# Pi-Star-Lab/RESCO

Hardware: AMD Instinct MI355X
Metric: env-steps/sec (higher is better)
Workload: dtype f32; 1 GPU; ingolstadt21 x 4096 lock-step envs per GPU (BASELINE config 3), fixed demand from the map's rou.xml, on-device seeded random policy, Krauss sigma 0.5 + speedFactor dev 0.1; tls_expiry=1, map=ingolstadt21, envs_per_gpu=4096, pipes=2, ticks_per_env_step=10, block_threads=512, lds_bytes_per_env=40896, parallelism=env-batch split x1, no collective on the data path

## Files before the change

resco_amd/csrc/resco_step.h:

```cpp
#pragma once
#include "resco_tables.h"

struct State {
    char *base;
    size_t nc;
    int32_t *trip_log;
    int32_t *env;
    int32_t *tls;
    long long *stats;
    uint16_t *dep_next;
    uint32_t *mail;
    RS_HD float *pos() const { return (float *)base; }
    RS_HD float *speed() const { return RS_G((float *)(base + 4 * nc)); }
    RS_HD float *accel() const { return RS_G((float *)(base + 8 * nc)); }
    RS_HD float *tloss() const { return RS_G((float *)(base + 12 * nc)); }
    RS_HD float *sf() const { return RS_G((float *)(base + 16 * nc)); }
    RS_HD uint32_t *coop(int par) const { return RS_G((uint32_t *)(base + (par ? 43 : 20) * nc)); }
    RS_HD uint32_t *cooplead(int par) const { return RS_G((uint32_t *)(base + (par ? 47 : 24) * nc)); }
    RS_HD uint16_t *lane() const { return RS_G((uint16_t *)(base + 28 * nc)); }
    RS_HD uint16_t *trip() const { return RS_G((uint16_t *)(base + 30 * nc)); }
    RS_HD uint16_t *cursor() const { return RS_G((uint16_t *)(base + 32 * nc)); }
    RS_HD uint16_t *swait() const { return RS_G((uint16_t *)(base + 34 * nc)); }
    RS_HD uint16_t *rwait() const { return RS_G((uint16_t *)(base + 36 * nc)); }
    RS_HD uint16_t *depart() const { return RS_G((uint16_t *)(base + 38 * nc)); }
// ... 345 lines not shown
    const int waves = C >= 768 ? 8 : ((C / 2) + 63) / 64;
    return (waves * 64 == 512 && lds <= RS_LDS_4WG_LIMIT) ? V64 : V80;
}
RS_CARVE void scn_consts_layout(ScnConsts *c, const Lds &L, size_t lds_bytes) {
#define X(n, tp) c->o_##n = L.n.off;
    RS_SCN_LDS(X)
#undef X
    c->gstride = L.gstride; c->lcap = L.lcap; c->lds_bytes = (uint32_t)lds_bytes;
    __builtin_memcpy(&c->cell_inv_bits, &L.cell_inv, 4);
}
template <class F> RS_CARVE bool scn_fix_matches(const ScnConsts &c) {
    bool ok = c.cell_inv_bits == F::cell_inv_bits && c.gstride == F::gstride && c.lcap == F::lcap && c.lds_bytes == F::lds_bytes && c.budget == F::budget;
#define X(n) ok = ok && c.n == F::n;
    RS_SCN_KTAB(X)
#undef X
#define X(n) ok = ok && c.n##_bits == F::n##_bits;
    RS_SCN_KTAB_F(X)
#undef X
#define X(n, tp) ok = ok && c.o_##n == F::o_##n;
    RS_SCN_LDS(X)
#undef X
    return ok;
}

struct StepArgs { KTab T; State G; Out O; Lds L; StateP GP; };

template <int DEM, class TT> struct Demand {
    const TT &T;
    const uint32_t off;
    RS_MEM Demand(const TT &T_, int env) : T(T_), off(DEM == 1 || (DEM == 2 && T_.dem()) ? rs_at(T_.dem_env(), env) : 0u) {}
    template <class Tp> RS_MEM const Tp *at(uint32_t o) const { return (const Tp *)(T.dem() + (off + o)); }
    RS_MEM const int32_t *trip_depart() const { if constexpr (DEM == 1) return at<int32_t>(dem_off_depart(T.n_trips, T.n_dep, T.horizon)); else if constexpr (DEM == 2) return T.dem() ? at<int32_t>(dem_off_depart(T.n_trips, T.n_dep, T.horizon)) : T.cold.trip_depart; else return T.cold.trip_depart; }
    RS_MEM const int32_t *trips_cum() const { if constexpr (DEM == 1) return at<int32_t>(dem_off_cum(T.n_trips, T.n_dep, T.horizon)); else if constexpr (DEM == 2) return T.dem() ? at<int32_t>(dem_off_cum(T.n_trips, T.n_dep, T.horizon)) : T.cold.trips_cum; else return T.cold.trips_cum; }
    RS_MEM const uint16_t *trip_next() const { if constexpr (DEM == 1) return at<uint16_t>(dem_off_next(T.n_trips, T.n_dep, T.horizon)); else if constexpr (DEM == 2) return T.dem() ? at<uint16_t>(dem_off_next(T.n_trips, T.n_dep, T.horizon)) : T.cold.trip_next; else return T.cold.trip_next; }
    RS_MEM const uint16_t *trip_route() const { if constexpr (DEM == 1) return at<uint16_t>(dem_off_route(T.n_trips, T.n_dep, T.horizon)); else if constexpr (DEM == 2) return T.dem() ? at<uint16_t>(dem_off_route(T.n_trips, T.n_dep, T.horizon)) : T.trip_route(); else return T.trip_route(); }
    RS_MEM const uint16_t *dep_first() const { if constexpr (DEM == 1) return at<uint16_t>(dem_off_first(T.n_trips, T.n_dep, T.horizon)); else if constexpr (DEM == 2) return T.dem() ? at<uint16_t>(dem_off_first(T.n_trips, T.n_dep, T.horizon)) : T.cold.dep_first; else return T.cold.dep_first; }
    RS_MEM const uint8_t *trip_vtype() const { if constexpr (DEM == 1) return at<uint8_t>(dem_off_vtype(T.n_trips, T.n_dep, T.horizon)); else if constexpr (DEM == 2) return T.dem() ? at<uint8_t>(dem_off_vtype(T.n_trips, T.n_dep, T.horizon)) : T.trip_vtype(); else return T.trip_vtype(); }
};

#ifndef RS_LAYOUT_ONLY
template <class F> struct KTabFix {
    const KTab &K;
    const KCold &cold;
    RS_MEM explicit KTabFix(const KTab &K_) : K(K_), cold(K_.cold) {}
#define X(n) static constexpr int32_t n = F::n;
    RS_SCN_KTAB(X)
#undef X
#define X(n) static constexpr float n = __builtin_bit_cast(float, (uint32_t)F::n##_bits);
    RS_SCN_KTAB_F(X)
#undef X
    RS_MEM const LaneRec *lanes() const { return K.lanes(); }
    RS_MEM const LinkRec *links() const { return K.links(); }
    RS_MEM const FoeRec *foes() const { return K.foes(); }
    RS_MEM const RStep *rsteps() const { return K.rsteps(); }
    RS_MEM const float *route_cont() const { return K.route_cont(); }
    RS_MEM const uint16_t *next_link() const { return K.next_link(); }
    RS_MEM const uint16_t *notbest() const { return K.notbest(); }
    RS_MEM const RouteRec *routes() const { return K.routes(); }
    RS_MEM const uint16_t *trip_route() const { return K.trip_route(); }
    RS_MEM const uint8_t *trip_vtype() const { return K.trip_vtype(); }
    RS_MEM const char *dem() const { return K.dem(); }
    RS_MEM const uint32_t *dem_env() const { return K.dem_env(); }
};
template <class F> struct LdsScn {
#define X(n, tp) CPtr<tp, F::o_##n> n;
    RS_SCN_LDS(X)
#undef X
    static constexpr uint32_t gstride = F::gstride, lcap = F::lcap;
    static constexpr float cell_inv = __builtin_bit_cast(float, (uint32_t)F::cell_inv_bits);
};

#ifdef RS_EMU_DEBUG
#define RS_CHAIN_GUARD if (++rs_dbg_chain > 50000000L) { printf("endless chain walk\n"); fflush(stdout); abort(); }
#else
#define RS_CHAIN_GUARD
#endif
#ifndef RS_ASSERT
#define RS_ASSERT(c)
#endif
#ifndef RS_SEC
#define RS_SEC_BEGIN
#define RS_SEC(id) {}
#endif
template <class LT> RS_DEV int lane_cells(const LT &L, const LaneRec &LR) { return (int)(LR.len * L.cell_inv) + 1; }
template <class LT> RS_DEV int cell_of(const LT &L, float pos, int ncell) { const int c = (int)(pos * L.cell_inv); return c < ncell ? c : ncell - 1; }

struct Grid { uint16_t *c; uint32_t tag; };
RS_DEV unsigned long long grid_tag4(const Grid &g) { return g.tag ? 0x8000800080008000ull : 0ull; }
RS_DEV int cell_head(const Grid &g, int c) {
    const uint32_t v = g.c[c];
    return ((v ^ g.tag) & CELL_TAG) ? (int)NIL : (int)(v & NIL);
}
RS_DEV uint16_t grid_push(const Grid &g, int c, int s, bool mover) {
    uint32_t *w = (uint32_t *)g.c + (c >> 1);
    const int sh = (c & 1) * 16;
    const uint32_t flag = (mover ? CELL_MOVER : 0u) | g.tag;
    uint32_t old = *w, assumed, cell;
    do {
        assumed = old;
        cell = (assumed >> sh) & 0xFFFFu;
        if ((cell ^ g.tag) & CELL_TAG) cell = NIL;
        const uint32_t keep = cell & CELL_MOVER;
        uint32_t cnt = (cell >> CELL_CNT_SHIFT) & CELL_CNT_MAX;
        if (cnt < CELL_CNT_MAX) cnt += 1u;
        old = rs_atomic_cas(w, assumed, (assumed & ~(0xFFFFu << sh)) | (((uint32_t)s | (cnt << CELL_CNT_SHIFT) | keep | flag) << sh));
    } while (old != assumed);
    return (uint16_t)(cell & NIL);
}
RS_DEV unsigned long long quad_load(const Grid &g, int b) { return *(const unsigned long long *)(g.c + b) ^ grid_tag4(g); }
RS_DEV unsigned long long quad_occ(const Grid &g, int b) {
    const unsigned long long w = quad_load(g, b);
    const unsigned long long x = (w & 0x07FF07FF07FF07FFull) ^ 0x07FF07FF07FF07FFull;
    return (x + 0x07FF07FF07FF07FFull) & 0x0800080008000800ull & ~(w >> 4);
}
RS_DEV int cells_count(const Grid &g, int c0, int nc) {
    const int c1 = c0 + nc - 1;
    int n = 0;
    for (int b = c0 & ~3; b <= c1; b += 4) {
        const unsigned long long w = quad_load(g, b);
        unsigned long long m = (w >> CELL_CNT_SHIFT) & 0x0007000700070007ull;
        m &= ~(((w >> 15) & 0x0001000100010001ull) * 7ull);
        const int lo = c0 - b, hi = c1 - b;
        if (lo > 0) m &= ~0ull << (16 * lo);
        if (hi < 3) m &= ~0ull >> (16 * (3 - hi));
        n += (int)((m * 0x0001000100010001ull) >> 48);
    }
    return n;
}
RS_DEV int scan_up(const Grid &g, int c0, int c1) {
    for (int b = c0 & ~3; b <= c1; b += 4) {
        unsigned long long m = quad_occ(g, b);
        const int lo = c0 - b, hi = c1 - b;
        if (lo > 0) m &= ~0ull << (16 * lo);
        if (hi < 3) m &= ~0ull >> (16 * (3 - hi));
        if (m) return b + ((rs_ffsll(m) - 1) >> 4);
    }
    return -1;
}
RS_DEV int scan_down(const Grid &g, int c0, int c1) {
    for (int b = c1 & ~3; b + 3 >= c0; b -= 4) {
        unsigned long long m = quad_occ(g, b);
        const int lo = c0 - b, hi = c1 - b;
        if (lo > 0) m &= ~0ull << (16 * lo);
        if (hi < 3) m &= ~0ull >> (16 * (3 - hi));
        if (m) return b + ((63 - rs_clzll(m)) >> 4);
        if (b == 0) break;
    }
    return -1;
}
RS_DEV bool cells_have_mover(const Grid &g, int c0, int nc) {
    const int c1 = c0 + nc - 1;
    for (int b = c0 & ~3; b <= c1; b += 4) {
        const unsigned long long w = quad_load(g, b);
        unsigned long long m = w & 0x4000400040004000ull & ~(w >> 1);
        const int lo = c0 - b, hi = c1 - b;
        if (lo > 0) m &= ~0ull << (16 * lo);
        if (hi < 3) m &= ~0ull >> (16 * (3 - hi));
        if (m) return true;
    }
    return false;
}
RS_DEV unsigned long long order_key(float pos, int trip) { return ((unsigned long long)(uint32_t)rs_float_as_int(pos) << 16) | (uint32_t)(0xFFFF - trip); }
RS_DEV float key_pos(unsigned long long key) { return rs_int_as_float((int)(uint32_t)(key >> 16)); }
#ifndef RS_KEEP4
#define RS_KEEP4(a, b, c, d)
#endif
// ... 31 lines not shown
template <class LT> RS_DEV Found chain_rearmost(const LT &L, int head) {
    Found f{(int)NIL, ~0ull, 0u, 0u};
    for (int s = head & NIL; s != NIL;) RS_CHAIN_STEP(f, s, key < f.key)
    return f;
}
template <class LT> RS_DEV Found chain_frontmost(const LT &L, int head) {
    Found f{(int)NIL, 0ull, 0u, 0u};
    for (int s = head & NIL; s != NIL;) RS_CHAIN_STEP(f, s, key > f.key)
    return f;
}
template <class LT> RS_DEV Found rearmost_within(const LT &L, const Grid &grid, int cell0, int ncell, float win) {
    Found f{(int)NIL, ~0ull, 0u, 0u};
    if (win < 0.0f) return f;
    const int c = scan_up(grid, cell0, cell0 + cell_of(L, win, ncell));
    if (c < 0) return f;
    f = chain_rearmost(L, cell_head(grid, c));
    if (f.slot != NIL && f.pos() > win) f.slot = NIL;
    return f;
}
template <class LT> RS_DEV Found leader_found(const LT &L, const Grid &grid, int cell0, int ncell, float pos, int k, int self, float win) {
    const int c = cell_of(L, pos, ncell);
    const unsigned long long mykey = order_key(pos, k);
    Found f{(int)NIL, ~0ull, 0u, 0u};
    const uint32_t cw = grid.c[cell0 + c];
    int s = ((cw ^ grid.tag) & CELL_TAG) ? (int)NIL : (int)(cw & NIL);
    if (s == self && ((cw >> CELL_CNT_SHIFT) & CELL_CNT_MAX) == 1u) s = NIL;
    while (s != NIL) {
        RS_ASSERT(s != self || order_key(L.node[s].pos, L.node[s].trip) == mykey)
        RS_CHAIN_STEP(f, s, (key > mykey) & (key < f.key))
    }
    if (f.slot == NIL && c + 1 < ncell) {
        const int cc = scan_up(grid, cell0 + c + 1, cell0 + cell_of(L, pos + win, ncell));
        if (cc >= 0) f = chain_rearmost(L, cell_head(grid, cc));
    }
    if (f.slot != NIL && f.pos() - pos > win) f.slot = NIL;
    return f;
}
template <class LT> RS_DEV int leader_within(const LT &L, const Grid &grid, int cell0, int ncell, float pos, int k, int self, float win) {
    return leader_found(L, grid, cell0, ncell, pos, k, self, win).slot;
}
template <class LT> RS_DEV int follower_within(const LT &L, const Grid &grid, int cell0, int ncell, float pos, int k, int self, float win) {
    const int c = cell_of(L, pos, ncell);
    const unsigned long long mykey = order_key(pos, k);
    Found f{(int)NIL, 0ull, 0u, 0u};
    for (int s = cell_head(grid, cell0 + c); s != NIL;) {
        RS_ASSERT(s != self || order_key(L.node[s].pos, L.node[s].trip) == mykey)
        RS_CHAIN_STEP(f, s, (key < mykey) & (key > f.key))
    }
    if (f.slot == NIL && c > 0) {
        const float lo = pos - win;
        const int cc = scan_down(grid, cell0 + (lo > 0.0f ? cell_of(L, lo, ncell) : 0), cell0 + c - 1);
        if (cc >= 0) f = chain_frontmost(L, cell_head(grid, cc));
    }
    if (f.slot != NIL && pos - f.pos() > win) f.slot = NIL;
    (void)self;
    return f.slot;
}
template <class LT> RS_DEV int at_or_behind_within(const LT &L, const Grid &grid, int cell0, int ncell, float back, float win) {
    if (back < 0.0f) return NIL;
    const int c = cell_of(L, back, ncell);
    Found f{(int)NIL, 0ull, 0u, 0u};
    for (int s = cell_head(grid, cell0 + c); s != NIL;) RS_CHAIN_STEP(f, s, !(nd_.pos > back) & (key > f.key))
    if (f.slot == NIL && c > 0) {
        const float lo = back - win;
        const int cc = scan_down(grid, cell0 + (lo > 0.0f ? cell_of(L, lo, ncell) : 0), cell0 + c - 1);
        if (cc >= 0) f = chain_frontmost(L, cell_head(grid, cc));
    }
    if (f.slot != NIL && back - f.pos() > win) f.slot = NIL;
    return f.slot;
}

template <class TT, class LT> RS_DEV int tls_state(const TT &T, const LT &L, int tls, int pos) {
    if (tls == 0xFF) return TLS_G;
    return L.tstate[tls * T.tls_maxl + pos];
}
template <class TT> RS_DEV uint16_t cache_link(const TT &T, const LaneRec &LR, int lane, int rq, int trip) {
    if (LR.link_cnt == 0) return NLINK_NONE;
    if (LR.flags & LF_INTERNAL) { const int l = LR.link_start; return (uint16_t)(l | (rs_at(T.links(), l).arr_idx >= 0 ? NLINK_ARR : 0)); }
    return rs_at(T.next_link(), ((uint32_t)rq * (uint32_t)T.kmax + (uint32_t)(lane - (int)LR.edge_lane0)) * 2u + (uint32_t)(trip & 1));
}
template <class TT, class LT> RS_DEV bool foe_blocked(const TT &T, const LT &L, const Grid &grid, const LinkRec &K) {
    for (int i = K.foe_start; i < K.foe_start + K.foe_cnt; ++i) {
        const FoeRec F = rec_load16(T.foes(), i);
        if (F.tls != 0xFF && tls_state(T, L, F.tls, F.tls_pos) == TLS_R) continue;
        if (F.arr_idx >= 0 && L.arr[F.arr_idx] < RM_FOE_GAP_Q) return true;
        if (F.via1_cell0 != 0xFFFF && cells_have_mover(grid, F.via1_cell0, F.via1_nc)) return true;
        if (F.via2_cell0 != 0xFFFF && cells_have_mover(grid, F.via2_cell0, F.via2_nc)) return true;
    }
    return false;
}
template <class TT, class LT> RS_DEV void tls_refresh(const TT &T, const LT &L, const KParams &P, int s, int ph) {
    const int w = T.tls_maxl >> 2;
    const uint32_t *src = (const uint32_t *)((P.fixed_program ? T.cold.fix8 + T.cold.fix_state_off[s] : T.cold.tls8 + T.cold.tls_state_off[s]) + ph * T.tls_maxl);
    uint32_t *dst = (uint32_t *)((uint8_t *)L.tstate + s * T.tls_maxl);
    uint32_t v[8];
#pragma unroll
    for (int i = 0; i < 8; ++i) v[i] = src[i < w ? i : 0];
#pragma unroll
    for (int i = 0; i < 8; ++i) if (i < w) dst[i] = v[i];
#pragma unroll 1
    for (int i = 8; i < w; ++i) dst[i] = src[i];
}
template <class TT, class LT> RS_DEV void set_phase(const TT &T, const LT &L, const KParams &P, int s, int ph) {
    if (ph < 0 || ph >= T.cold.tls_nphase[s]) return;
    L.phase[s] = ph;
    L.left[s] = P.tls_expiry ? T.cold.tls_dur[T.cold.tls_dur_off[s] + ph] : RM_TLS_HOLD_TICKS;
    tls_refresh(T, L, P, s, ph);
}
template <class TT, class LT> RS_DEV void tls_begin_of_tick(const TT &T, const LT &L, const KParams &P, int s, int tick) {
    if (P.do_fsm && !P.fixed_program && tick == T.yellow_length) set_phase(T, L, P, s, L.nextp[s]);
    int left = L.left[s];
    if (left == 0) {
        const int32_t *dur = P.fixed_program ? T.cold.fix_dur + T.cold.fix_dur_off[s] : T.cold.tls_dur + T.cold.tls_dur_off[s];
        const int Pn = P.fixed_program ? T.cold.fix_nphase[s] : T.cold.tls_nphase[s];
        const int ph = (L.phase[s] + 1) % Pn;
        left = dur[ph];
        L.phase[s] = ph;
        tls_refresh(T, L, P, s, ph);
    }
    L.left[s] = left - 1;
}
struct ContRow { float c[4]; const float *cn; };
template <class TT> RS_DEV ContRow cont_row(const TT &T, int rq) {
    ContRow R;
    R.cn = (const float *)((const char *)T.route_cont() + (uint32_t)rq * (uint32_t)T.kmax * 4u);
    for (int j = 0; j < 4; ++j) R.c[j] = j < T.kmax ? R.cn[j] : 0.0f;
    return R;
}
RS_DEV float cont_of(const ContRow &R, int j) {
    return j == 0 ? R.c[0] : (j == 1 ? R.c[1] : (j == 2 ? R.c[2] : (j == 3 ? R.c[3] : R.cn[j])));
}
#define OCC_NONE (Grid{(uint16_t *)0, 0u})
#define OCC_FULL (Grid{(uint16_t *)1, 0u})
RS_DEV bool cont_notbest(float c) { return rs_float_as_int(c) < 0; }
RS_DEV float cont_len(float c) { return rs_int_as_float(rs_float_as_int(c) & 0x7FFFFFFF); }
RS_DEV int strategic_dir(const ContRow &R, int kk, int n, float x, float v, int extra, float &rem, const Grid &grid, int cell0, int nc, float occ_unit) {
    const float mine = cont_of(R, kk);
    rem = cont_len(mine) - x;
#ifdef RS_EMU_CHECK_MAIL
    { float best = 0.0f; for (int j = 0; j < n; ++j) { const float c = cont_len(cont_of(R, j)); if (c > best) best = c; }
      for (int j = 0; j < n; ++j) RS_ASSERT(cont_notbest(cont_of(R, j)) == !(cont_len(cont_of(R, j)) >= best - RM_CONT_EPS)) }
#endif
    if (!cont_notbest(mine)) return 0;
    int dl = 1000, dr = 1000;
    for (int j = kk + 1; j < n; ++j) if (!cont_notbest(cont_of(R, j))) { dl = j - kk; break; }
    for (int j = kk - 1; j >= 0; --j) if (!cont_notbest(cont_of(R, j))) { dr = kk - j; break; }
    const int dir = (dr <= dl) ? -1 : +1;
    if (grid.c == (uint16_t *)1) return dir;
    const int off = (dr <= dl ? dr : dl) + extra;
    const float la = (v > RM_LOOK_MIN_SPEED ? v : RM_LOOK_MIN_SPEED) * RM_LOOK_TIME + RM_LOOK_BASE;
    int cnt = 0;
    if (grid.c != (uint16_t *)0) cnt = cells_count(grid, cell0 + ((dr <= dl) ? -dr : dl) * nc, nc);
    if (rem - (float)cnt * occ_unit >= la * (float)off) return 0;
    return dir;
}
template <class TT> RS_DEV uint32_t link_reg_word(const TT &T, int nlk) { return rs_at((const uint32_t *)T.links(), (uint32_t)(nlk & 0x7FFF) * 8u + 2u); }
template <class TT, class LT> RS_DEV void register_approach_w(const TT &T, const LT &L, uint32_t kw, float v, float pos, float lane_len, int vt) {
    const int st = tls_state(T, L, (int)((kw >> 16) & 0xFFu), (int)(kw >> 24));
    if (st == TLS_R) return;
    const float dist = lane_len - pos;
    if (st == TLS_Y && dist >= d_brake_gap(v, L.vtp[vt * VT_COLS + VT_DECEL])) return;
    const float ta = RS_DIV(dist, v > 1.0f ? v : 1.0f);
    const int q = ta * 10.0f >= 65000.0f ? 65000 : (int)(ta * 10.0f);
    rs_atomic_min(&L.arr[(int16_t)(kw & 0xFFFFu)], q);
}
template <class TT, class LT> RS_DEV void register_approach(const TT &T, const LT &L, int nlk, float v, float pos, float lane_len, int vt) {
    if (!(nlk & NLINK_ARR)) return;
    if (v <= RM_HALT_SPEED) return;
    register_approach_w(T, L, link_reg_word(T, nlk), v, pos, lane_len, vt);
}
template <class TT, class LT> RS_DEV void follow_neighbour(const TT &T, const LT &L, uint32_t key, bool clamp_gap, const LaneRec &LR, int lane, float x, float v,
                             float b, float tau, float mingap, float &vsafe) {
    const int X = (int)(key & 0xFFFFu), kx = (int)(key >> 16);
    if ((int)L.node[X].trip != kx) return;
    const int lx = L.aux[X].lane;
    if (lx == (int)LANE_NONE || (LR.flags & LF_INTERNAL)) return;
    const int l0 = LR.edge_lane0, n = LR.flags >> 2;
    if (lx < l0 || lx >= l0 + n) return;
    const float *vo = L.vtp + L.node[X].vt * VT_COLS;
    const float px = L.node[X].pos, backx = px - vo[VT_LENGTH];
    if (clamp_gap ? !(px >= x) : !(backx >= x)) return;
    float g = backx - x - mingap;
    if (clamp_gap && g < 0.0f) g = 0.0f;
    float vs = d_follow_speed(g, L.node[X].speed, b, vo[VT_DECEL], tau);
    float vc = v - b; if (vc < 0.0f) vc = 0.0f;
    if (vs < vc) vs = vc;
    if (vs < vsafe) vsafe = vs;
    (void)lane;
}

template <class LT> RS_DEV void mail_flag_set(const LT &L, int s, int par) { rs_atomic_or((uint32_t *)((Node *)L.node + s) + 3, SFQ_MAIL(par) << 16); }
template <class LT> RS_DEV void mail_flag_clear(const LT &L, int s, int par) { rs_atomic_and((uint32_t *)((Node *)L.node + s) + 3, ~(SFQ_MAIL(par) << 16)); }
template <class LT, class LP> RS_DEV void list_push(const LT &L, const LP &list, int counter, int s);
template <class LT> RS_DEV void flag_mover(const LT &L, int s, int t, int lct = 0) {
    uint32_t *w = (uint32_t *)((Node *)L.node + s) + 3;
    const uint32_t bit = (uint32_t)fl_mh(t) << 8;
    if (!(rs_atomic_fetch_or(w, bit | ((uint32_t)lct << 8)) & bit)) list_push(L, L.ls_mh, SC_NMH + (t & 1), s);
}
template <class LT, class LP> RS_DEV void list_push(const LT &L, const LP &list, int counter, int s) {
    const int i = rs_wave_ticket(&L.sc[counter]);
    if (i < (int)L.lcap) list[i] = (uint16_t)s;
}
RS_DEV float plan_vfree(const float *vt, float v, float lane_vmax, float sf) {
    float vfree = v + vt[VT_ACCEL];
    const float vl = lane_vmax * sf;
    if (vl < vfree) vfree = vl;
    if (vt[VT_MAXSPEED] < vfree) vfree = vt[VT_MAXSPEED];
    return vfree;
}
RS_DEV float plan_look(const float *vt, float vfree) { return d_brake_gap(vfree, vt[VT_DECEL]) + vfree * vt[VT_TAU] + vt[VT_MINGAP] + 1.0f; }
RS_DEV bool looks_beyond(const float *vt, float v, float x, float lane_len, float lane_vmax, float sf) {
    return lane_len - x < plan_look(vt, plan_vfree(vt, v, lane_vmax, sf));
}
RS_DEV bool may_change_lanes_row(const ContRow &R, const LaneRec &LR, int lane, int k, float x, float v, int t) {
    const int n = LR.flags >> 2;
    if ((LR.flags & LF_INTERNAL) || n < 2) return false;
    const int kk = lane - (int)LR.edge_lane0;
    float rem;
    if (strategic_dir(R, kk, n, x, v, 0, rem, OCC_FULL, 0, 0, 0.0f) != 0) return true;
    if ((((uint32_t)t >> 1) + (uint32_t)k) & 3u) return false;
    const int tk = kk + ((t & 1) ? -1 : +1);
    return tk >= 0 && tk < n && strategic_dir(R, tk, n, x, v, RM_SG_EXTRA_LANES, rem, OCC_NONE, 0, 0, 0.0f) == 0;
}
template <class TT> RS_DEV bool may_change_lanes(const TT &T, int rq, uint32_t nb, const LaneRec &LR, int lane, int k, float x, float v, int t) {
    const int n = LR.flags >> 2;
    if ((LR.flags & LF_INTERNAL) || n < 2) return false;
    const int kk = lane - (int)LR.edge_lane0;
    bool r;
    if ((nb >> kk) & 1u) r = true;
    else if ((((uint32_t)t >> 1) + (uint32_t)k) & 3u) r = false;
    else {
        const int tk = kk + ((t & 1) ? -1 : +1);
        if (tk < 0 || tk >= n) r = false;
        else if (!((nb >> tk) & 1u)) r = true;
        else { float rem; r = strategic_dir(cont_row(T, rq), tk, n, x, v, RM_SG_EXTRA_LANES, rem, OCC_NONE, 0, 0, 0.0f) == 0; }
    }
#ifdef RS_EMU_CHECK_MAIL
    RS_ASSERT(r == may_change_lanes_row(cont_row(T, rq), LR, lane, k, x, v, t))
#endif
    return r;
}
template <class TT, class LT> RS_DEV int classify(const TT &T, const LT &L, int s, const float *vt, float v, float x, const LaneRec &LR, int lane, int rq, uint32_t nb, int k, float sf, int t) {
    int fl = 0;
    if (looks_beyond(vt, v, x, LR.len, LR.vmax, sf)) { fl |= FL_H; list_push(L, L.ls_h, SC_NH, s); }
    if (may_change_lanes(T, rq, nb, LR, lane, k, x, v, t)) { fl |= FL_LC; list_push(L, L.ls_lc, SC_NLC, s); }
    return fl;
}

template <bool LONG, class TT, class LT, class GT> RS_DEV void phase_plan(const TT &T, const LT &L, const Grid &grid, const GT &G, size_t eo, const KParams &P, int genv, int t, int s) {
    RS_SEC_BEGIN
    const Aux ax = L.aux[s];
    const int lane = ax.lane;
    if (lane == (int)LANE_NONE) return;
    const Node me = L.node[s];
    const int k = me.trip;
    const float *vt = L.vtp + me.vt * VT_COLS;
    const float a = vt[VT_ACCEL], b = vt[VT_DECEL], tau = vt[VT_TAU], mingap = vt[VT_MINGAP];
    const float v = me.speed, x = me.pos;
    const float sf = sf_of(me.sfq);
    const LaneRec LR0 = rec_load16(T.lanes(), lane);
    LaneRec LR = LR0;
    float vsafe = RM_BIGF;
    float tgap = 0.0f, tvl = 0.0f, tbl = b;
    bool have = false;
    if (LONG) RS_SEC(7)
    const float vfree = plan_vfree(vt, v, LR.vmax, sf);
    const float look = plan_look(vt, vfree);
    const Found ld = leader_found(L, grid, LR.cell0, lane_cells(L, LR), x, k, s, look + T.maxlen);
    const int lead = ld.slot;
    if (LONG) RS_SEC(8)
    bool found = false;
    if (lead != NIL) {
        const float *vo = L.vtp + ld.vt() * VT_COLS;
        tgap = ld.pos() - vo[VT_LENGTH] - x - mingap;
        tvl = ld.speed(); tbl = vo[VT_DECEL];
        have = true; found = true;
    }
    if (me.sfq & SFQ_MAIL((t + 1) & 1)) {
        const int q = (t + 1) & 1;
        const uint32_t c1 = G.coop(q)[eo + s], c2 = G.cooplead(q)[eo + s];
        if (c1 != COOP_NONE) { G.coop(q)[eo + s] = COOP_NONE; follow_neighbour(T, L, c1, false, LR, lane, x, v, b, tau, mingap, vsafe); }
        if (c2 != COOP_NONE) { G.cooplead(q)[eo + s] = COOP_NONE; follow_neighbour(T, L, c2, true, LR, lane, x, v, b, tau, mingap, vsafe); }
        mail_flag_clear(L, s, q);
    }
#ifdef RS_EMU_CHECK_MAIL
    else { RS_ASSERT(G.coop((t + 1) & 1)[eo + s] == COOP_NONE && G.cooplead((t + 1) & 1)[eo + s] == COOP_NONE) }
#endif
    if (LONG) RS_SEC(9)
    float seen = LR.len - x;
    RS_ASSERT(LONG || found || !(seen < look))
    if (LONG && !found && seen < look) {
        int rq = ax.rq;
        int link = (int)(ax.nlink & 0x7FFF);
        int cur_lane = lane;
        const float bgv = d_brake_gap(v, b);
        for (int hop = 0; hop < RM_MAX_HOPS; ++hop) {
            const bool cur_int = (LR.flags & LF_INTERNAL) != 0;
            if (hop > 0) link = (int)(cache_link(T, LR, cur_lane, rq, k) & 0x7FFF);
            bool stop_here = false;
            LinkRec K;
            if (link == NLINK_NONE) {
                if (!cur_int && rs_at(T.rsteps(), rq).next_edge == 0xFFFF) break;
                stop_here = true;
            } else {
                K = link_load(T.links(), link);
                const int st = tls_state(T, L, K.tls, K.tls_pos);
                if (K.tls != 0xFF && (st == TLS_R || st == TLS_Y) && seen >= bgv) stop_here = true;
                if (!stop_here && !(K.flags & KF_CONT) && ((K.flags & KF_MINOR) || (K.tls != 0xFF && st == TLS_g))) {
                    if (seen > RM_VIS_DIST) stop_here = true;
                    else if (K.foe_cnt > 0 && foe_blocked(T, L, grid, K)) stop_here = true;
                }
            }
            if (stop_here) {
                const float g = seen - RM_STOP_OFFSET;
                tgap = g > 0.0f ? g : 0.0f; tvl = 0.0f; tbl = b;
                have = true;
                break;
            }
            LR = K.dest;
            cur_lane = K.to_lane;
            {
                const float vnl = LR.vmax * sf;
                if (vnl < vfree) {
                    const float vs = d_free_speed(seen, vnl, b);
                    if (vs < vsafe) vsafe = vs;
                }
            }
            const Found od = rearmost_within(L, grid, LR.cell0, lane_cells(L, LR), look - seen + T.maxlen);
            if (od.slot != NIL) {
                const float *vo = L.vtp + od.vt() * VT_COLS;
                tgap = seen + od.pos() - vo[VT_LENGTH] - mingap;
                tvl = od.speed(); tbl = vo[VT_DECEL];
                have = true;
                break;
            }
            if (!cur_int) rq += 1;
            seen += LR.len;
            if (!(seen < look)) break;
        }
    }
    if (LONG) RS_SEC(10)
    if (have) {
        const float vs = d_follow_speed(tgap, tvl, b, tbl, tau);
        if (vs < vsafe) vsafe = vs;
    }
    float vmin_n = v - b; if (vmin_n < 0.0f) vmin_n = 0.0f;
    float vmin_e = v - vt[VT_EMERGENCY]; if (vmin_e < 0.0f) vmin_e = 0.0f;
    const float lo = vsafe > vmin_e ? vsafe : vmin_e;
    const float vmin = vmin_n < lo ? vmin_n : lo;
    float vmax = vfree < vsafe ? vfree : vsafe;
    if (vmax < vmin) vmax = vmin;
    const float sigma = P.sigma >= 0.0f ? P.sigma : vt[VT_SIGMA];
    float vd = vmax;
    if (sigma > 0.0f) {
        const float r = d_u01(d_hash(P.seed, (uint32_t)genv, (uint32_t)k, (uint32_t)t, 0u));
        if (vd < a) vd -= sigma * vd * r; else vd -= sigma * a * r;
        if (vd < 0.0f) vd = 0.0f;
    }
    const float vnext = vd > vmin ? vd : vmin;
    L.vnx[s] = vnext;
#ifdef RS_EMU_DEBUG
    if (s == rs_dbg_slot && (t == rs_dbg_t || rs_dbg_t < 0))
        printf("plan t %d slot %d lane %d x %.3f v %.3f lead %d have %d tgap %.3f tvl %.3f vsafe %.3f vfree %.3f vnext %.3f nlink %x\n", t, s, lane, x, v, lead,
               (int)have, tgap, tvl, vsafe, vfree, vnext, ax.nlink);
#endif
    if (LONG) RS_SEC(3)
    if (x + vnext > LR0.len) flag_mover(L, s, t);
    if (LONG) RS_SEC(15)
    (void)LR;
}

template <bool LONG, class TT, class LT, class GT> RS_DEV void phase_move(const TT &T, const LT &L, const Grid &gnew, const GT &G, const KParams &P, int env, size_t eo,
                       int t, bool last_tick, bool more, int s, int &active, int &halted, int &top) {
    const Aux ax = L.aux[s];
    const Node me = L.node[s];
    const int k = me.trip;
    int lane = ax.lane;
#ifdef RS_EMU_DEBUG
    {
        static int moved_at[65536];
        if (moved_at[s] == t + 1) { printf("slot %d moved twice in tick %d: fl %x lane %d trip %d\n", s, t, me.fl, lane, k); fflush(stdout); abort(); }
        moved_at[s] = t + 1;
    }
#endif
#ifdef RS_FIELD_LOADS
    LaneRec LR = rec_load16(T.lanes(), lane);
#endif
    uint32_t nb = rs_at(T.notbest(), ax.rq);
    uint32_t kw = 0;
    if (more && (ax.nlink & NLINK_ARR)) kw = link_reg_word(T, ax.nlink);
    const float sfv = sf_of(me.sfq);
    float tl = G.tloss()[eo + s];
#ifndef RS_FIELD_LOADS
    LaneRec LR = rec_load16(T.lanes(), lane);
#endif
    const int sw = ax.swait;
    int swn = sw;
    const float vn = L.vnx[s];
    int rq = ax.rq;
    uint16_t nlink = ax.nlink;
    int link = (int)(nlink & 0x7FFF);
    bool relink = false;
    int side = 0;
    RS_ASSERT(LONG || (!(me.fl & (LCT_LEFT | LCT_RIGHT | LCT_SWAP_LEFT | LCT_SWAP_RIGHT)) && !(me.pos + vn > LR.len)))
    if (LONG && (me.fl & (LCT_LEFT | LCT_RIGHT | LCT_SWAP_LEFT | LCT_SWAP_RIGHT))) {
        if ((me.fl & (LCT_LEFT | LCT_RIGHT)) && !(me.pos + vn > LR.len)) side = (me.fl & LCT_LEFT) ? +1 : -1;
        else if (me.fl & (LCT_SWAP_LEFT | LCT_SWAP_RIGHT)) side = (me.fl & LCT_SWAP_LEFT) ? +1 : -1;
    }
    if (LONG && side) {
        lane += side;
        LR = rec_load16(T.lanes(), lane);
        nlink = cache_link(T, LR, lane, rq, k);
        link = (int)(nlink & 0x7FFF);
        relink = true;
    }
    const float vref = LR.vmax * sfv;
    if (last_tick && (P.out_mask & OUT_VEH_ACCEL)) G.accel()[eo + s] = vn - me.speed;
    if (vn <= RM_HALT_SPEED) {
        if (sw < 65535) swn = sw + 1;
        halted += 1;
        if (G.trip_log) { const int wt = G.wtot()[eo + s]; if (wt < 65535) G.wtot()[eo + s] = (uint16_t)(wt + 1); }
    } else swn = 0;
    if (vref > 0.0f && vn < vref) { tl += RS_DIV(vref - vn, vref); G.tloss()[eo + s] = tl; }
    float x = me.pos + vn;
    bool arrived = false;
    if (LONG) for (int it = 0; it < 16; ++it) {
        if (!(x > LR.len)) break;
        const bool li = (LR.flags & LF_INTERNAL) != 0;
        if (link == NLINK_NONE) {
            if (!li && rs_at(T.rsteps(), rq).next_edge == 0xFFFF) arrived = true; else x = LR.len;
            break;
        }
        x -= LR.len;
        if (!li) rq += 1;
        {
            const LinkRec Km = link_load(T.links(), link);
            lane = Km.to_lane;
            LR = Km.dest;
        }
        nlink = cache_link(T, LR, lane, rq, k);
        link = (int)(nlink & 0x7FFF);
        relink = true;
    }
    if (LONG && arrived) {
        Aux na = ax; na.lane = LANE_NONE; na.swait = 0;
        L.aux[s] = na;
        L.node[s].trip = TRIP_NONE; L.node[s].fl = (uint8_t)(me.fl & fl_mh(t));
        rs_atomic_and(&L.alive[s >> 5], ~(1u << (s & 31)));
        {
            const int ow = G.owner()[eo + s];
            if (ow != (int)OWNER_NONE) rs_atomic_add(&L.sig_dep[ow], 1);
        }
        G.owner()[eo + s] = OWNER_NONE; G.rwait()[eo + s] = 0;
        rs_atomic_add(&L.sc[SC_NACT], -1);
        rs_atomic_add(&L.sc[SC_STATS + ST_ARRIVED], 1);
        rs_atomic_add(&L.sc[SC_STATS + ST_DURATION], t + 1 - (int)G.depart()[eo + s]);
        rs_atomic_add(&L.sc[SC_STATS + ST_TLOSS], (int)(tl * 1024.0f + 0.5f));
        if (G.trip_log) {
            int32_t *r = G.trip_log + ((size_t)env * T.n_trips + k) * 4;
            r[0] = (int)G.depart()[eo + s]; r[1] = t + 1; r[2] = (int)(tl * 1024.0f + 0.5f); r[3] = (int)G.wtot()[eo + s];
        }
        return;
    }
    active += 1;
    if (s + 1 > top) top = s + 1;
    Aux na = ax;
    na.lane = (uint16_t)lane; na.rq = (uint16_t)rq; na.swait = (uint16_t)swn;
    if (LONG && relink) na.nlink = nlink;
    L.aux[s] = na;
    Node nn = me;
    nn.pos = x; nn.speed = vn; nn.fl = (uint8_t)(me.fl & fl_mh(t));
    nn.nxt = grid_push(gnew, LR.cell0 + cell_of(L, x, lane_cells(L, LR)), s, vn > RM_HALT_SPEED);
    if (more) {
        if (LONG && relink) { nb = rs_at(T.notbest(), rq); if (na.nlink & NLINK_ARR) kw = link_reg_word(T, na.nlink); }
        nn.fl |= classify(T, L, s, L.vtp + me.vt * VT_COLS, vn, x, LR, lane, rq, nb, k, sfv, t + 1);
        L.node[s] = nn;
        if ((na.nlink & NLINK_ARR) && vn > RM_HALT_SPEED) register_approach_w(T, L, kw, vn, x, LR.len, me.vt);
    } else L.node[s] = nn;
    (void)P;
}

template <class LT> RS_DEV int overlapping(const LT &L, const Grid &grid, int cell0, int ncell, float pos, int k, int self, float len_self) {
    const int lead = leader_within(L, grid, cell0, ncell, pos, k, self, RM_NB_WINDOW);
    if (lead != NIL && L.node[lead].pos - L.vtp[L.node[lead].vt * VT_COLS + VT_LENGTH] - pos < 0.0f) return lead;
    const int foll = follower_within(L, grid, cell0, ncell, pos, k, self, RM_NB_WINDOW);
    if (foll != NIL && pos - len_self - L.node[foll].pos < 0.0f) return foll;
    return NIL;
}

template <class TT, class LT, class GT> RS_DEV int phase_lc_decide(const TT &T, const LT &L, const Grid &grid, const GT &G, size_t eo, int t, int s, const Aux &ax, const Node &me) {
    const int lane = ax.lane;
#ifdef RS_FIELD_LOADS
    const LaneRec LR = rec_load16(T.lanes(), lane);
    const ContRow R = cont_row(T, ax.rq);
#else
    const ContRow R = cont_row(T, ax.rq);
    const LaneRec LR = rec_load16(T.lanes(), lane);
#endif
    const int my_wait = (int)ax.swait;
    const int n = LR.flags >> 2;
    if ((LR.flags & LF_INTERNAL) || n < 2) return 0;
    const int dir_allowed = (t & 1) ? -1 : +1;
    const int l0 = LR.edge_lane0, kk = lane - l0;
    const int k = me.trip;
    const float *vt = L.vtp + me.vt * VT_COLS;
    const float x = me.pos, v = me.speed;
    const int nc = lane_cells(L, LR);
    int want = 0, dir = dir_allowed;
    float rem;
    const int sdir = strategic_dir(R, kk, n, x, v, 0, rem, grid, LR.cell0, nc, T.occ_unit);
    if (sdir != 0) { dir = sdir; want = 2; }
    int code = 0;
    const int tk = kk + dir;
    if (tk >= 0 && tk < n) {
        const int tcell0 = (int)LR.cell0 + dir * nc;
        int lead_t = NIL, foll_t = NIL;
        bool have_t = false;
        if (!want && !((((uint32_t)t >> 1) + (uint32_t)k) & 3u)) {
            float rem_t;
            if (strategic_dir(R, tk, n, x, v, RM_SG_EXTRA_LANES, rem_t, grid, tcell0, nc, T.occ_unit) == 0) {
                const int lead_c = leader_within(L, grid, LR.cell0, nc, x, k, s, RM_NB_WINDOW);
                if (lead_c != NIL) {
                    lead_t = leader_within(L, grid, tcell0, nc, x, k, s, RM_NB_WINDOW);
                    have_t = true;
                    const float gcur = L.node[lead_c].pos - L.vtp[L.node[lead_c].vt * VT_COLS + VT_LENGTH] - x;
                    float gtgt = RM_BIGF;
                    if (lead_t != NIL) gtgt = L.node[lead_t].pos - L.vtp[L.node[lead_t].vt * VT_COLS + VT_LENGTH] - x;
                    if (gcur < v * 3.0f + 15.0f && gtgt > gcur + RM_SG_ADVANTAGE) want = 1;
                }
            }
        }
        if (want) {
            if (!have_t) lead_t = leader_within(L, grid, tcell0, nc, x, k, s, RM_NB_WINDOW);
            foll_t = follower_within(L, grid, tcell0, nc, x, k, s, RM_NB_WINDOW);
            const bool urgent = want == 2 && rem <= RM_URGENT_DIST;
            bool safe = true;
            if (lead_t != NIL) {
                const Node ld = L.node[lead_t];
                const float *vo = L.vtp + ld.vt * VT_COLS;
                const float gap = ld.pos - vo[VT_LENGTH] - x - (urgent ? 0.0f : vt[VT_MINGAP]);
                const float dec = urgent ? vt[VT_EMERGENCY] : vt[VT_DECEL];
                float vb = v - dec; if (vb < 0.0f) vb = 0.0f;
                if (gap < 0.0f || vb > d_follow_speed(gap, ld.speed, vt[VT_DECEL], vo[VT_DECEL], vt[VT_TAU])) safe = false;
            }
            if (safe && foll_t != NIL) {
                const Node fd = L.node[foll_t];
                const float *vo = L.vtp + fd.vt * VT_COLS;
                const float gap = x - vt[VT_LENGTH] - fd.pos - (urgent ? 0.0f : vo[VT_MINGAP]);
                const float dec = urgent ? vo[VT_EMERGENCY] : vo[VT_DECEL];
                float vb = fd.speed - dec; if (vb < 0.0f) vb = 0.0f;
                if (gap < 0.0f || vb > d_follow_speed(gap, v, vo[VT_DECEL], vt[VT_DECEL], vo[VT_TAU])) safe = false;
            }
            if (safe) {
                if (dir == dir_allowed) code = dir > 0 ? LCT_LEFT : LCT_RIGHT;
            } else if (want == 2) {
                if (lead_t != NIL) { G.cooplead(t & 1)[eo + s] = ((uint32_t)L.node[lead_t].trip << 16) | (uint32_t)lead_t; mail_flag_set(L, s, t & 1); }
                const int R = at_or_behind_within(L, grid, tcell0, nc, x - vt[VT_LENGTH], RM_COOP_RANGE);
                if (R != NIL) { rs_atomic_min(&G.coop(t & 1)[eo + R], ((uint32_t)k << 16) | (uint32_t)s); mail_flag_set(L, R, t & 1); }
            }
        }
    }
    if (sdir != 0 && (t % RM_SWAP_EVERY) == 0 && v <= RM_HALT_SPEED && rem <= RM_URGENT_DIST &&
        my_wait >= RM_SWAP_WAIT) {
        const int b = overlapping(L, grid, (int)LR.cell0 + sdir * nc, nc, x, k, s, vt[VT_LENGTH]);
        if (b != NIL) {
            const Node nb = L.node[b];
            float rem_b;
            if (nb.speed <= RM_HALT_SPEED && (int)L.aux[b].swait >= RM_SWAP_WAIT &&
                strategic_dir(cont_row(T, L.aux[b].rq), kk + sdir, n, nb.pos, nb.speed, 0, rem_b, grid, (int)LR.cell0 + sdir * nc, nc, T.occ_unit) == -sdir && rem_b <= RM_URGENT_DIST &&
                overlapping(L, grid, LR.cell0, nc, nb.pos, nb.trip, b, L.vtp[nb.vt * VT_COLS + VT_LENGTH]) == s)
                code |= sdir > 0 ? LCT_SWAP_LEFT : LCT_SWAP_RIGHT;
        }
    }
        return code;
}

template <class TT, class DT, class LT> RS_DEV bool phase_insert_decide(const TT &T, const DT &D, const LT &L, const Grid &grid, int t, int d) {
    if ((int)L.dep_t[d] > t) return false;
    const int k = L.dep[d];
    const DepInfo LR = rec_load8(T.cold.dep_info, d);
    const float *vt = L.vtp + rs_at(D.trip_vtype(), k) * VT_COLS;
    const float mypos = vt[VT_LENGTH] < LR.len ? vt[VT_LENGTH] : LR.len;
    const int nc = (int)(LR.len * L.cell_inv) + 1;
    const int c1 = LR.cell0 + cell_of(L, mypos + vt[VT_MINGAP] + T.maxlen, nc);
    for (int c = scan_up(grid, LR.cell0, c1); c >= 0; c = (c < c1 ? scan_up(grid, c + 1, c1) : -1))
        for (int o = cell_head(grid, c); o != NIL;) { RS_CHAIN_GUARD
            const Node od = L.node[o];
            const float back = (od.pos + L.vnx[o]) - L.vtp[od.vt * VT_COLS + VT_LENGTH];
            if (back - mypos - vt[VT_MINGAP] < 0.0f) return false;
            o = od.nxt;
        }
    return true;
}

template <class LT> RS_DEV int nth_free_slot(const LT &L, int C, int r) {
#pragma unroll 1
    for (int w = 0; w < (C + 31) / 32; ++w) {
        uint32_t fr = ~L.alive0[w];
        if (w == (C - 1) / 32 && (C & 31)) fr &= (1u << (C & 31)) - 1u;
        const int c = rs_popc(fr);
        if (r >= c) { r -= c; continue; }
#pragma unroll 1
        for (int j = 0; j < r; ++j) fr &= fr - 1u;
        return w * 32 + rs_ffs(fr) - 1;
    }
    return -1;
}

template <class TT, class LT, class GT> RS_DEV void lc_decide_and_flag(const TT &T, const LT &L, const Grid &grid, const GT &G, size_t eo, int t, int s) {
    const Aux ax = L.aux[s];
    if (ax.lane == LANE_NONE) return;
    const int code = phase_lc_decide(T, L, grid, G, eo, t, s, ax, L.node[s]);
    if (code) flag_mover(L, s, t, code);
}
struct ExecInline {};

template <int CAP, bool DEM, class Exec, class LT, class TT, class GT>
RS_DEV void rs_step_body_on(Exec &ex, const LT &L, const TT &T, const GT &G, const Out &O, const KParams &P,
                            const int32_t *actions, int env) {
#ifdef RS_DEM_RUNTIME
    const Demand<2, TT> D(T, env);
#else
    const Demand<DEM, TT> D(T, env);
#endif
    const int B = ex.B;
    const int C = CAP ? CAP : T.capacity, S = T.n_signals, NO = T.n_obs;
    const int genv = P.env_base + env;
    const size_t eo = (size_t)env * C;
    const int n_ticks = P.n_ticks;

    uint16_t *const grid0 = L.grid;

    ex.phase(0, [&](int tid) {
        if (tid < SC_STATS + ST_N) L.sc[tid] = tid < 4 ? G.env[env * 4 + tid] : 0;
        for (int i = tid; i < T.n_vtypes * VT_COLS; i += B) L.vtp[i] = T.cold.vtype_params[i];
        for (int i = tid; i < (int)(L.gstride >> 1); i += B) ((uint32_t *)grid0)[i] = 0x07FF07FFu;
        for (int i = tid; i < T.n_arr; i += B) L.arr[i] = ARR_NONE;
        for (int i = tid; i < (C + 31) / 32; i += B) { L.alive[i] = 0u; L.mailw[i] = 0u; }
        for (int i = tid; i < (T.n_dep + 31) / 32; i += B) L.insm[i] = 0u;
        for (int i = tid; i < T.n_dep; i += B) {
            const int k = G.dep_next[(size_t)env * T.n_dep + i];
            L.dep[i] = (uint16_t)k;
            L.dep_t[i] = k == (int)TRIP_NONE ? (uint16_t)0xFFFF : (uint16_t)D.trip_depart()[k];
        }
        for (int i = tid; i < S; i += B) {
            const int ph = G.tls[(env * S + i) * TLS_W + 0];
            L.phase[i] = ph;
            L.left[i] = G.tls[(env * S + i) * TLS_W + 1];
            L.nextp[i] = G.tls[(env * S + i) * TLS_W + 2];
            L.sig_arr[i] = 0; L.sig_dep[i] = G.tls[(env * S + i) * TLS_W + 3];
            tls_refresh(T, L, P, i, ph);
        }
    });
    ex.phase(1, [&](int tid) {
// ... 351 lines not shown
```

Measured before the change: 4.238 million env-steps/s.

## Use precomputed notbest bitmasks, branchless lookahead walk, and unify leader lookups

Replaces the per-lane scan loops in strategic_dir with a precomputed not-best bitmask and uses ffs/clz to find the nearest best lane. The lookahead hop loop becomes predicated straight-line code with a go flag instead of early breaks, which should reduce branch divergence across wavefront lanes. The lane-change decision is reorganised so the target-lane leader lookup happens once on a shared path. Debug counters are added as no-op macros. The cost is unconditional link and tls-state loads on every hop, plus a new dependency on the T.notbest() table.

```diff
diff --git a/resco_amd/csrc/resco_step.h b/resco_amd/csrc/resco_step.h
--- a/resco_amd/csrc/resco_step.h
+++ b/resco_amd/csrc/resco_step.h
@@ -451,6 +451,14 @@
 #define RS_SEC_BEGIN
 #define RS_SEC(id) {}
 #endif
+enum RsCount {
+    RC_WALK, RC_HOP2, RC_HOP3, RC_HOP4, RC_MAX_HOPS, RC_ROUTE_END, RC_DEAD_END, RC_STOP_RED, RC_RED_TOO_CLOSE, RC_MINOR_FAR,
+    RC_FOE_IN, RC_FOE_BLOCKED, RC_FOE_RED, RC_FOE_ARR, RC_FOE_VIA1, RC_FOE_VIA2, RC_NEXT_LEADER, RC_LOOK_DONE,
+    RC_STRATEGIC, RC_SG, RC_SG_LEAD, RC_SG_WANT, RC_URGENT, RC_FOLL_T, RC_CHANGE, RC_LEAD_REQ, RC_COOP_REQ, RC_SWAP, RC_COUNT
+};
+#ifndef RS_COUNT
+#define RS_COUNT(id) {}
+#endif
 template <class LT> RS_DEV int lane_cells(const LT &L, const LaneRec &LR) { return (int)(LR.len * L.cell_inv) + 1; }
 template <class LT> RS_DEV int cell_of(const LT &L, float pos, int ncell) { const int c = (int)(pos * L.cell_inv); return c < ncell ? c : ncell - 1; }
 
@@ -648,10 +656,10 @@
 template <class TT, class LT> RS_DEV bool foe_blocked(const TT &T, const LT &L, const Grid &grid, const LinkRec &K) {
     for (int i = K.foe_start; i < K.foe_start + K.foe_cnt; ++i) {
         const FoeRec F = rec_load16(T.foes(), i);
-        if (F.tls != 0xFF && tls_state(T, L, F.tls, F.tls_pos) == TLS_R) continue;
-        if (F.arr_idx >= 0 && L.arr[F.arr_idx] < RM_FOE_GAP_Q) return true;
-        if (F.via1_cell0 != 0xFFFF && cells_have_mover(grid, F.via1_cell0, F.via1_nc)) return true;
-        if (F.via2_cell0 != 0xFFFF && cells_have_mover(grid, F.via2_cell0, F.via2_nc)) return true;
+        if (F.tls != 0xFF && tls_state(T, L, F.tls, F.tls_pos) == TLS_R) { RS_COUNT(RC_FOE_RED) continue; }
+        if (F.arr_idx >= 0 && L.arr[F.arr_idx] < RM_FOE_GAP_Q) { RS_COUNT(RC_FOE_ARR) return true; }
+        if (F.via1_cell0 != 0xFFFF && cells_have_mover(grid, F.via1_cell0, F.via1_nc)) { RS_COUNT(RC_FOE_VIA1) return true; }
+        if (F.via2_cell0 != 0xFFFF && cells_have_mover(grid, F.via2_cell0, F.via2_nc)) { RS_COUNT(RC_FOE_VIA2) return true; }
     }
     return false;
 }
@@ -700,17 +708,20 @@
 #define OCC_FULL (Grid{(uint16_t *)1, 0u})
 RS_DEV bool cont_notbest(float c) { return rs_float_as_int(c) < 0; }
 RS_DEV float cont_len(float c) { return rs_int_as_float(rs_float_as_int(c) & 0x7FFFFFFF); }
-RS_DEV int strategic_dir(const ContRow &R, int kk, int n, float x, float v, int extra, float &rem, const Grid &grid, int cell0, int nc, float occ_unit) {
+RS_DEV uint32_t row_notbest(const ContRow &R, int n) { uint32_t nb = 0; for (int j = 0; j < n; ++j) nb |= cont_notbest(cont_of(R, j)) ? 1u << j : 0u; return nb; }
+RS_DEV int strategic_dir(const ContRow &R, uint32_t nb, int kk, int n, float x, float v, int extra, float &rem, const Grid &grid, int cell0, int nc, float occ_unit) {
     const float mine = cont_of(R, kk);
     rem = cont_len(mine) - x;
 #ifdef RS_EMU_CHECK_MAIL
     { float best = 0.0f; for (int j = 0; j < n; ++j) { const float c = cont_len(cont_of(R, j)); if (c > best) best = c; }
-      for (int j = 0; j < n; ++j) RS_ASSERT(cont_notbest(cont_of(R, j)) == !(cont_len(cont_of(R, j)) >= best - RM_CONT_EPS)) }
-#endif
-    if (!cont_notbest(mine)) return 0;
-    int dl = 1000, dr = 1000;
-    for (int j = kk + 1; j < n; ++j) if (!cont_notbest(cont_of(R, j))) { dl = j - kk; break; }
-    for (int j = kk - 1; j >= 0; --j) if (!cont_notbest(cont_of(R, j))) { dr = kk - j; break; }
+      for (int j = 0; j < n; ++j) RS_ASSERT(cont_notbest(cont_of(R, j)) == !(cont_len(cont_of(R, j)) >= best - RM_CONT_EPS))
+      RS_ASSERT((nb & ((1u << n) - 1u)) == row_notbest(R, n)) }
+#endif
+    if (!((nb >> kk) & 1u)) return 0;
+    const uint32_t good = ~nb & ((1u << n) - 1u);
+    const uint32_t up = good >> (kk + 1), dn = good & ((1u << kk) - 1u);
+    const int dl = up ? rs_ffs(up) : 1000;
+    const int dr = dn ? kk - (63 - rs_clzll((unsigned long long)dn | 1ull)) : 1000;
     const int dir = (dr <= dl) ? -1 : +1;
     if (grid.c == (uint16_t *)1) return dir;
     const int off = (dr <= dl ? dr : dl) + extra;
@@ -783,10 +794,11 @@
     if ((LR.flags & LF_INTERNAL) || n < 2) return false;
     const int kk = lane - (int)LR.edge_lane0;
     float rem;
-    if (strategic_dir(R, kk, n, x, v, 0, rem, OCC_FULL, 0, 0, 0.0f) != 0) return true;
+    const uint32_t nb = row_notbest(R, n);
+    if (strategic_dir(R, nb, kk, n, x, v, 0, rem, OCC_FULL, 0, 0, 0.0f) != 0) return true;
     if ((((uint32_t)t >> 1) + (uint32_t)k) & 3u) return false;
     const int tk = kk + ((t & 1) ? -1 : +1);
-    return tk >= 0 && tk < n && strategic_dir(R, tk, n, x, v, RM_SG_EXTRA_LANES, rem, OCC_NONE, 0, 0, 0.0f) == 0;
+    return tk >= 0 && tk < n && strategic_dir(R, nb, tk, n, x, v, RM_SG_EXTRA_LANES, rem, OCC_NONE, 0, 0, 0.0f) == 0;
 }
 template <class TT> RS_DEV bool may_change_lanes(const TT &T, int rq, uint32_t nb, const LaneRec &LR, int lane, int k, float x, float v, int t) {
     const int n = LR.flags >> 2;
@@ -799,7 +811,7 @@
         const int tk = kk + ((t & 1) ? -1 : +1);
         if (tk < 0 || tk >= n) r = false;
         else if (!((nb >> tk) & 1u)) r = true;
-        else { float rem; r = strategic_dir(cont_row(T, rq), tk, n, x, v, RM_SG_EXTRA_LANES, rem, OCC_NONE, 0, 0, 0.0f) == 0; }
+        else { float rem; r = strategic_dir(cont_row(T, rq), nb, tk, n, x, v, RM_SG_EXTRA_LANES, rem, OCC_NONE, 0, 0, 0.0f) == 0; }
     }
 #ifdef RS_EMU_CHECK_MAIL
     RS_ASSERT(r == may_change_lanes_row(cont_row(T, rq), LR, lane, k, x, v, t))
@@ -860,50 +872,65 @@
         int link = (int)(ax.nlink & 0x7FFF);
         int cur_lane = lane;
         const float bgv = d_brake_gap(v, b);
-        for (int hop = 0; hop < RM_MAX_HOPS; ++hop) {
+        RS_COUNT(RC_WALK)
+        bool go = true;
+        for (int hop = 0; go && hop < RM_MAX_HOPS; ++hop) {
+            if (hop == 1) RS_COUNT(RC_HOP2)
+            if (hop == 2) RS_COUNT(RC_HOP3)
+            if (hop >= 3) RS_COUNT(RC_HOP4)
             const bool cur_int = (LR.flags & LF_INTERNAL) != 0;
             if (hop > 0) link = (int)(cache_link(T, LR, cur_lane, rq, k) & 0x7FFF);
-            bool stop_here = false;
-            LinkRec K;
-            if (link == NLINK_NONE) {
-                if (!cur_int && rs_at(T.rsteps(), rq).next_edge == 0xFFFF) break;
-                stop_here = true;
-            } else {
-                K = link_load(T.links(), link);
-                const int st = tls_state(T, L, K.tls, K.tls_pos);
-                if (K.tls != 0xFF && (st == TLS_R || st == TLS_Y) && seen >= bgv) stop_here = true;
-                if (!stop_here && !(K.flags & KF_CONT) && ((K.flags & KF_MINOR) || (K.tls != 0xFF && st == TLS_g))) {
-                    if (seen > RM_VIS_DIST) stop_here = true;
-                    else if (K.foe_cnt > 0 && foe_blocked(T, L, grid, K)) stop_here = true;
+            const bool none = link == NLINK_NONE;
+            const LinkRec K = link_load(T.links(), none ? 0 : link);
+            const bool sig = !none & (K.tls != 0xFF);
+            const int st0 = L.tstate[sig ? K.tls * T.tls_maxl + K.tls_pos : 0];
+            const int st = sig ? st0 : (int)TLS_G;
+            bool route_end = false;
+            if (none) route_end = !cur_int && rs_at(T.rsteps(), rq).next_edge == 0xFFFF;
+            const bool red = (st == TLS_R) | (st == TLS_Y);
+            const bool red_stop = red & (seen >= bgv);
+            const bool minor = !none & !red_stop & !(K.flags & KF_CONT) & (((K.flags & KF_MINOR) != 0) | (st == TLS_g));
+            const bool far = minor & (seen > RM_VIS_DIST);
+            bool stop_here = (none & !route_end) | red_stop | far;
+            if (none & route_end) RS_COUNT(RC_ROUTE_END)
+            if (none & !route_end) RS_COUNT(RC_DEAD_END)
+            if (red_stop) RS_COUNT(RC_STOP_RED)
+            if (red & !red_stop) RS_COUNT(RC_RED_TOO_CLOSE)
+            if (far) RS_COUNT(RC_MINOR_FAR)
+            if (minor && !far && K.foe_cnt > 0) {
+                RS_COUNT(RC_FOE_IN)
+                if (foe_blocked(T, L, grid, K)) { RS_COUNT(RC_FOE_BLOCKED) stop_here = true; }
+            }
+            {
+                const float g = seen - RM_STOP_OFFSET;
+                tgap = stop_here ? (g > 0.0f ? g : 0.0f) : tgap; tvl = stop_here ? 0.0f : tvl; tbl = stop_here ? b : tbl;
+            }
+            const bool cont = !none & !stop_here;
+            bool hit = false;
+            if (cont) {
+                LR = K.dest;
+                cur_lane = K.to_lane;
+                {
+                    const float vnl = LR.vmax * sf;
+                    if (vnl < vfree) {
+                        const float vs = d_free_speed(seen, vnl, b);
+                        if (vs < vsafe) vsafe = vs;
+                    }
                 }
-            }
-            if (stop_here) {
-                const float g = seen - RM_STOP_OFFSET;
-                tgap = g > 0.0f ? g : 0.0f; tvl = 0.0f; tbl = b;
-                have = true;
-                break;
-            }
-            LR = K.dest;
-            cur_lane = K.to_lane;
-            {
-                const float vnl = LR.vmax * sf;
-                if (vnl < vfree) {
-                    const float vs = d_free_speed(seen, vnl, b);
-                    if (vs < vsafe) vsafe = vs;
-                }
-            }
-            const Found od = rearmost_within(L, grid, LR.cell0, lane_cells(L, LR), look - seen + T.maxlen);
-            if (od.slot != NIL) {
+                const Found od = rearmost_within(L, grid, LR.cell0, lane_cells(L, LR), look - seen + T.maxlen);
+                hit = od.slot != NIL;
                 const float *vo = L.vtp + od.vt() * VT_COLS;
-                tgap = seen + od.pos() - vo[VT_LENGTH] - mingap;
-                tvl = od.speed(); tbl = vo[VT_DECEL];
-                have = true;
-                break;
-            }
-            if (!cur_int) rq += 1;
-            seen += LR.len;
-            if (!(seen < look)) break;
-        }
+                tgap = hit ? seen + od.pos() - vo[VT_LENGTH] - mingap : tgap;
+                tvl = hit ? od.speed() : tvl; tbl = hit ? vo[VT_DECEL] : tbl;
+                rq += cur_int ? 0 : 1;
+                seen += LR.len;
+            }
+            have |= stop_here | hit;
+            if (hit) RS_COUNT(RC_NEXT_LEADER)
+            if (cont & !hit & !(seen < look)) RS_COUNT(RC_LOOK_DONE)
+            go = cont & !hit & (seen < look);
+        }
+        if (go) RS_COUNT(RC_MAX_HOPS)
     }
     if (LONG) RS_SEC(10)
     if (have) {
@@ -1063,6 +1090,7 @@
     const ContRow R = cont_row(T, ax.rq);
     const LaneRec LR = rec_load16(T.lanes(), lane);
 #endif
+    const uint32_t nbm = rs_at(T.notbest(), ax.rq);
     const int my_wait = (int)ax.swait;
     const int n = LR.flags >> 2;
     if ((LR.flags & LF_INTERNAL) || n < 2) return 0;
@@ -1074,32 +1102,34 @@
     const int nc = lane_cells(L, LR);
     int want = 0, dir = dir_allowed;
     float rem;
-    const int sdir = strategic_dir(R, kk, n, x, v, 0, rem, grid, LR.cell0, nc, T.occ_unit);
-    if (sdir != 0) { dir = sdir; want = 2; }
+    const int sdir = strategic_dir(R, nbm, kk, n, x, v, 0, rem, grid, LR.cell0, nc, T.occ_unit);
+    if (sdir != 0) { RS_COUNT(RC_STRATEGIC) dir = sdir; want = 2; }
     int code = 0;
     const int tk = kk + dir;
     if (tk >= 0 && tk < n) {
         const int tcell0 = (int)LR.cell0 + dir * nc;
         int lead_t = NIL, foll_t = NIL;
-        bool have_t = false;
+        bool sg = false;
         if (!want && !((((uint32_t)t >> 1) + (uint32_t)k) & 3u)) {
             float rem_t;
-            if (strategic_dir(R, tk, n, x, v, RM_SG_EXTRA_LANES, rem_t, grid, tcell0, nc, T.occ_unit) == 0) {
-                const int lead_c = leader_within(L, grid, LR.cell0, nc, x, k, s, RM_NB_WINDOW);
-                if (lead_c != NIL) {
-                    lead_t = leader_within(L, grid, tcell0, nc, x, k, s, RM_NB_WINDOW);
-                    have_t = true;
-                    const float gcur = L.node[lead_c].pos - L.vtp[L.node[lead_c].vt * VT_COLS + VT_LENGTH] - x;
-                    float gtgt = RM_BIGF;
-                    if (lead_t != NIL) gtgt = L.node[lead_t].pos - L.vtp[L.node[lead_t].vt * VT_COLS + VT_LENGTH] - x;
-                    if (gcur < v * 3.0f + 15.0f && gtgt > gcur + RM_SG_ADVANTAGE) want = 1;
-                }
-            }
+            sg = strategic_dir(R, nbm, tk, n, x, v, RM_SG_EXTRA_LANES, rem_t, grid, tcell0, nc, T.occ_unit) == 0;
+        }
+        int lead_c = NIL;
+        if (sg) { RS_COUNT(RC_SG) lead_c = leader_within(L, grid, LR.cell0, nc, x, k, s, RM_NB_WINDOW); }
+        const bool sgl = sg && lead_c != NIL;
+        if (want || sgl) lead_t = leader_within(L, grid, tcell0, nc, x, k, s, RM_NB_WINDOW);
+        if (sgl) {
+            RS_COUNT(RC_SG_LEAD)
+            const float gcur = L.node[lead_c].pos - L.vtp[L.node[lead_c].vt * VT_COLS + VT_LENGTH] - x;
+            float gtgt = RM_BIGF;
+            if (lead_t != NIL) gtgt = L.node[lead_t].pos - L.vtp[L.node[lead_t].vt * VT_COLS + VT_LENGTH] - x;
+            if (gcur < v * 3.0f + 15.0f && gtgt > gcur + RM_SG_ADVANTAGE) { RS_COUNT(RC_SG_WANT) want = 1; }
         }
         if (want) {
-            if (!have_t) lead_t = leader_within(L, grid, tcell0, nc, x, k, s, RM_NB_WINDOW);
             foll_t = follower_within(L, grid, tcell0, nc, x, k, s, RM_NB_WINDOW);
             const bool urgent = want == 2 && rem <= RM_URGENT_DIST;
+            if (urgent) RS_COUNT(RC_URGENT)
+            if (foll_t != NIL) RS_COUNT(RC_FOLL_T)
             bool safe = true;
             if (lead_t != NIL) {
                 const Node ld = L.node[lead_t];
@@ -1118,11 +1148,11 @@
                 if (gap < 0.0f || vb > d_follow_speed(gap, v, vo[VT_DECEL], vt[VT_DECEL], vo[VT_TAU])) safe = false;
             }
             if (safe) {
-                if (dir == dir_allowed) code = dir > 0 ? LCT_LEFT : LCT_RIGHT;
+                if (dir == dir_allowed) { RS_COUNT(RC_CHANGE) code = dir > 0 ? LCT_LEFT : LCT_RIGHT; }
             } else if (want == 2) {
-                if (lead_t != NIL) { G.cooplead(t & 1)[eo + s] = ((uint32_t)L.node[lead_t].trip << 16) | (uint32_t)lead_t; mail_flag_set(L, s, t & 1); }
+                if (lead_t != NIL) { RS_COUNT(RC_LEAD_REQ) G.cooplead(t & 1)[eo + s] = ((uint32_t)L.node[lead_t].trip << 16) | (uint32_t)lead_t; mail_flag_set(L, s, t & 1); }
                 const int R = at_or_behind_within(L, grid, tcell0, nc, x - vt[VT_LENGTH], RM_COOP_RANGE);
-                if (R != NIL) { rs_atomic_min(&G.coop(t & 1)[eo + R], ((uint32_t)k << 16) | (uint32_t)s); mail_flag_set(L, R, t & 1); }
+                if (R != NIL) { RS_COUNT(RC_COOP_REQ) rs_atomic_min(&G.coop(t & 1)[eo + R], ((uint32_t)k << 16) | (uint32_t)s); mail_flag_set(L, R, t & 1); }
             }
         }
     }
@@ -1133,9 +1163,9 @@
             const Node nb = L.node[b];
             float rem_b;
             if (nb.speed <= RM_HALT_SPEED && (int)L.aux[b].swait >= RM_SWAP_WAIT &&
-                strategic_dir(cont_row(T, L.aux[b].rq), kk + sdir, n, nb.pos, nb.speed, 0, rem_b, grid, (int)LR.cell0 + sdir * nc, nc, T.occ_unit) == -sdir && rem_b <= RM_URGENT_DIST &&
+                strategic_dir(cont_row(T, L.aux[b].rq), rs_at(T.notbest(), L.aux[b].rq), kk + sdir, n, nb.pos, nb.speed, 0, rem_b, grid, (int)LR.cell0 + sdir * nc, nc, T.occ_unit) == -sdir && rem_b <= RM_URGENT_DIST &&
                 overlapping(L, grid, LR.cell0, nc, nb.pos, nb.trip, b, L.vtp[nb.vt * VT_COLS + VT_LENGTH]) == s)
-                code |= sdir > 0 ? LCT_SWAP_LEFT : LCT_SWAP_RIGHT;
+                { RS_COUNT(RC_SWAP) code |= sdir > 0 ? LCT_SWAP_LEFT : LCT_SWAP_RIGHT; }
         }
     }
         return code;
```

Result: faster. 4.403 million env-steps/s, median of 6 (+3.9%).
